# SZU-AdvTech-2024/140-ExtDM-Distribution-Extrapolation-Diffusion-Model-for-Video-Prediction

Hardware: NVIDIA B200
Metric: predicted frames/sec (DDIM, SMMNIST/BAIR 64²) at 1/2/4/8 B200; roofline % (higher is better)
Workload: dtype bf16

## Files before the change

### 140-extdm-distribution-extrapolation-diffusion-model-for-video-prediction_b200/csrc/conv_gemm.cu

```cuda
#include "common.cuh"
#include "../../include/extdm_b200.h"

#include <mutex>
#include <stdio.h>
#include <stdlib.h>
#include <string.h>

namespace extdm {

constexpr int kTileM = 128;
constexpr int kBlockK = 64;
constexpr int kATileBytes = kTileM * kBlockK * 2;
constexpr int kGemmThreads = 192;

struct GemmDev {
  int nk0, nk1, ntaps;
  int box[4], start[4], count[4], ntile[4];
  signed char tap[64][4];
  int n;
  int n_tiles_n, total_tiles;
  void* out;
  int out_fp32;
  long long out_base, out_stride[4];
  int col_group;
  long long col_group_stride;
  const float* bias;
  const void* res;
  int res_fp32;
  long long res_base, res_stride[4];
  const float* col_scale;
  const float* col_shift;
  int act;
  float* gn_part;
  int kh, kw, stages, a_ext_bytes;
  int n_phase;
  long long phase_out[4];
  int tf32;
  int prefetch;
  int dbg;
};

__device__ __forceinline__ float apply_act(float v, int act) {
  if (act == 1) return fmaxf(v, 0.0f);
  if (act == 2) return silu(v);
  if (act == 3) return 1.0f / (1.0f + __expf(-v));
  return v;
}

struct TileCoord {
  int c1, c2, c3, c4, n0, m_tile, phase;
};
__device__ __forceinline__ TileCoord decode_tile(const GemmDev& p, int tile, int BN) {
  TileCoord t;
  const int nt = tile % p.n_tiles_n;
// ... 217 lines not shown
      }
    }
    tc_fence_before();
    __syncwarp();
    if (lane == 0) mbar_arrive(&acc_empty[as]);

    if (GN) {
      asm volatile("bar.sync 1, 128;" ::: "memory");
      if (m < 16)
        p.gn_part[static_cast<long long>(tc.m_tile) * 16 + m] = (sg[m] + sg[16 + m]) + (sg[32 + m] + sg[48 + m]);
    }
  }
}


template <int BN, bool GN, int EPW, int NACC = 2>
__device__ __forceinline__ void epilogue_simple(const GemmDev& p, uint64_t* acc_full, uint64_t* acc_empty, float* s_gn,
                                                uint32_t tmem_base, int warp, int lane) {
  constexpr uint32_t kAccCols = BN < 32 ? 32 : BN;
  constexpr int kChunks = BN / 16;
  constexpr int kGroups = EPW >= NACC ? NACC : (EPW >= 2 ? 2 : 1);
  constexpr int kWpg = EPW / kGroups;
  constexpr int kGThreads = 128 * kWpg;
  const int q = warp & 3;
  const int e = (warp - 2) >> 2;
  const int grp = e / kWpg, eg = e % kWpg;
  float* s_bias = s_gn + grp * 256;
  const int gt = (eg * 4 + ((warp - 2) & 3)) * 32 + lane;
  const int m = q * 32 + lane;
  int r = m;
  const int i1 = r % p.box[0]; r /= p.box[0];
// ... 21 lines not shown
    }
    mbar_wait(&acc_full[as], aphase);
    tc_fence_after();
    const uint32_t taddr = tmem_base + as * kAccCols + (static_cast<uint32_t>(q * 32) << 16);
#pragma unroll 1
    for (int ch = eg; ch < kChunks; ch += kWpg) {
      uint32_t raw[16];
      if (p.dbg & 8) {
#pragma unroll
        for (int j = 0; j < 16; ++j) raw[j] = 0u;
      } else {
        tmem_ld16(taddr + ch * 16, raw);
        tmem_ld_wait();
      }
      float gst[4] = {0.f, 0.f, 0.f, 0.f};
      if (row_ok && n0 + ch * 16 < p.n) {
        float v[16];
#pragma unroll
        for (int j = 0; j < 16; j += 4) {
          const float4 bb = *reinterpret_cast<const float4*>(s_bias + ch * 16 + j);
          v[j] = __uint_as_float(raw[j]) + bb.x; v[j + 1] = __uint_as_float(raw[j + 1]) + bb.y;
          v[j + 2] = __uint_as_float(raw[j + 2]) + bb.z; v[j + 3] = __uint_as_float(raw[j + 3]) + bb.w;
        }
        if (p.act) {
#pragma unroll
          for (int j = 0; j < 16; ++j) v[j] = apply_act(v[j], p.act);
        }
        uint32_t pk[8];
#pragma unroll
        for (int j = 0; j < 8; ++j) pk[j] = pack_bf16(v[2 * j], v[2 * j + 1]);
        if (!(p.dbg & 1)) {
          *reinterpret_cast<uint4*>(orow + ch * 16) = make_uint4(pk[0], pk[1], pk[2], pk[3]);
          *reinterpret_cast<uint4*>(orow + ch * 16 + 8) = make_uint4(pk[4], pk[5], pk[6], pk[7]);
        }
        if (GN) {
#pragma unroll
          for (int j = 0; j < 8; ++j) {
            const float2 f = unpack_bf16(pk[j]);
            gst[j >> 2] += f.x + f.y;
            gst[2 + (j >> 2)] += f.x * f.x + f.y * f.y;
          }
        }
      }
      if (GN && !(p.dbg & 16)) {
        {
          const bool up = (lane & 16) != 0;
          const float s0 = up ? gst[0] : gst[2], k0 = up ? gst[2] : gst[0];
          const float s1 = up ? gst[1] : gst[3], k1 = up ? gst[3] : gst[1];
          gst[0] = k0 + __shfl_xor_sync(0xffffffffu, s0, 16);
          gst[1] = k1 + __shfl_xor_sync(0xffffffffu, s1, 16);
        }
        {
          const bool up = (lane & 8) != 0;
          const float s0 = up ? gst[0] : gst[1], k0 = up ? gst[1] : gst[0];
          gst[0] = k0 + __shfl_xor_sync(0xffffffffu, s0, 8);
        }
        gst[0] += __shfl_xor_sync(0xffffffffu, gst[0], 4);
        gst[0] += __shfl_xor_sync(0xffffffffu, gst[0], 2);
        gst[0] += __shfl_xor_sync(0xffffffffu, gst[0], 1);
        const int cpg = p.n >> 3;
        const int krec = cpg >= 32 ? (cpg >> 4) : 1;
        const int gcol = n0 + ch * 16;
        float* rec = p.gn_part + ((static_cast<long long>(tc.m_tile) * 4 + q) * krec + ((gcol >> 4) & (krec - 1))) * 16;
        const int stat = lane >> 4;
        if (cpg == 8) {
          if ((lane & 7) == 0) rec[stat * 8 + (gcol >> 3) + ((lane >> 3) & 1)] = gst[0];
        } else {
          const float tot = gst[0] + __shfl_xor_sync(0xffffffffu, gst[0], 8);
          if ((lane & 15) == 0) rec[stat * 8 + gcol / cpg] = tot;
        }
      }
    }
    tc_fence_before();
    __syncwarp();
    if (lane == 0) mbar_arrive(&acc_empty[as]);
  }
}

template <int BN, bool SIMPLE>
struct PlainCfg {
  static constexpr int kEpw = SIMPLE ? (BN == 256 ? 4 : 2) : 1;
  static constexpr int kThreads = 64 + 128 * kEpw;
};

template <int BN, int STAGES, bool GN, bool SIMPLE, bool TF32 = false>
__global__ void __launch_bounds__(PlainCfg<BN, SIMPLE>::kThreads, BN == 256 ? 1 : 2)
conv_gemm_kernel(const __grid_constant__ CUtensorMap map_a0, const __grid_constant__ CUtensorMap map_a1,
                 const __grid_constant__ CUtensorMap map_b, const __grid_constant__ GemmDev p) {
  constexpr int kBTileBytes = BN * kBlockK * 2;
  constexpr int kStageBytes = kATileBytes + kBTileBytes;
  constexpr uint32_t kAccCols = BN < 32 ? 32 : BN;
  constexpr uint32_t kTmemCols = 2 * kAccCols;

  extern __shared__ uint8_t smem_raw[];
  uint8_t* smem = reinterpret_cast<uint8_t*>((reinterpret_cast<uintptr_t>(smem_raw) + 1023) & ~uintptr_t(1023));
  uint64_t* full_bar = reinterpret_cast<uint64_t*>(smem + STAGES * kStageBytes);
  uint64_t* empty_bar = full_bar + STAGES;
  uint64_t* acc_full = empty_bar + STAGES;
  uint64_t* acc_empty = acc_full + 2;
  uint32_t* tmem_slot = reinterpret_cast<uint32_t*>(acc_empty + 2);
// ... 95 lines not shown
              for (int k = 0; k < kBlockK / 16; ++k) {
                if (TF32) umma_tf32(tmem_d, da + 2 * k, db + 2 * k, idesc, (it > 0 || k > 0) ? 1u : 0u);
                else umma_bf16(tmem_d, da + 2 * k, db + 2 * k, idesc, (it > 0 || k > 0) ? 1u : 0u);
              }
            }
            umma_commit(&empty_bar[stage]);
          }
          if (++stage == STAGES) { stage = 0; phase ^= 1; }
        }
        if (elect_one()) umma_commit(&acc_full[as]);
      }
    }
    __syncwarp();
  } else {
    if constexpr (SIMPLE)
      epilogue_simple<BN, GN, PlainCfg<BN, SIMPLE>::kEpw>(p, acc_full, acc_empty, s_gn, tmem_base, warp, lane);
    else
      epilogue_loop<BN, GN, false>(p, acc_full, acc_empty, s_gn, tmem_base, warp, lane);
  }

  tc_fence_before();
  __syncthreads();
  if (warp == 1) {
    tc_fence_after();
    tmem_dealloc(tmem_base, kTmemCols);
  }
}


constexpr int kHaloEpw = 4;
constexpr int kHaloThreads = 64 + 128 * kHaloEpw;

template <int BN, bool GN, bool RESB, bool SIMPLE>
__global__ void __launch_bounds__(SIMPLE ? kHaloThreads : kGemmThreads, 1)
conv_halo_kernel(const __grid_constant__ CUtensorMap map_a0, const __grid_constant__ CUtensorMap map_a1,
                 const __grid_constant__ CUtensorMap map_b, const __grid_constant__ GemmDev p) {
  constexpr int kBTileBytes = BN * kBlockK * 2;
  constexpr uint32_t kAccCols = BN < 32 ? 32 : BN;
  constexpr int kAcc = SIMPLE ? (BN <= 64 ? 4 : (BN <= 128 ? 4 : 2)) : 2;
  constexpr uint32_t kTmemCols = kAcc * kAccCols;
  static_assert(kTmemCols <= 512, "TMEM budget");
  constexpr int kMaxStages = 8;

  extern __shared__ uint8_t smem_raw[];
  uint8_t* smem = reinterpret_cast<uint8_t*>((reinterpret_cast<uintptr_t>(smem_raw) + 1023) & ~uintptr_t(1023));
  const int nk = p.nk0 + p.nk1;
  const int ntaps = p.kh * p.kw;
  const int resb_bytes = RESB ? ntaps * nk * kBTileBytes : 0;
// ... 122 lines not shown
                  acc = 1;
                }
              }
              if (p.dbg & 32) mbar_arrive(&empty_bar[stage]); else umma_commit(&empty_bar[stage]);
            }
            accumulate = 1;
            if (++stage == p.stages) { stage = 0; phase ^= 1; }
          }
        }
        if (elect_one()) { if (p.dbg & 32) mbar_arrive(&acc_full[as]); else umma_commit(&acc_full[as]); }
      }
    }
    __syncwarp();
  } else {
    if constexpr (SIMPLE)
      epilogue_simple<BN, GN, kHaloEpw, kAcc>(p, acc_full, acc_empty, s_gn, tmem_base, warp, lane);
    else
      epilogue_loop<BN, GN, false>(p, acc_full, acc_empty, s_gn, tmem_base, warp, lane);
  }

  tc_fence_before();
  __syncthreads();
  if (warp == 1) {
    tc_fence_after();
    tmem_dealloc(tmem_base, kTmemCols);
  }
}

typedef CUresult (*EncodeTiledFn)(CUtensorMap*, CUtensorMapDataType, cuuint32_t, void*, const cuuint64_t*,
                                  const cuuint64_t*, const cuuint32_t*, const cuuint32_t*, CUtensorMapInterleave,
                                  CUtensorMapSwizzle, CUtensorMapL2promotion, CUtensorMapFloatOOBfill);
// ... 35 lines not shown
static int encode_a(CUtensorMap* map, const void* base, int channels, const long long* dim, const long long* stride,
                    const int* box) {
  cuuint64_t dims[5] = {(cuuint64_t)channels, (cuuint64_t)dim[0], (cuuint64_t)dim[1], (cuuint64_t)dim[2],
                        (cuuint64_t)dim[3]};
  cuuint64_t strides[4] = {(cuuint64_t)stride[0] * 2, (cuuint64_t)stride[1] * 2, (cuuint64_t)stride[2] * 2,
                           (cuuint64_t)stride[3] * 2};
  cuuint32_t bx[5] = {(cuuint32_t)kBlockK, (cuuint32_t)box[0], (cuuint32_t)box[1], (cuuint32_t)box[2],
                      (cuuint32_t)box[3]};
  return encode_map(map, base, 5, dims, strides, bx, CU_TENSOR_MAP_L2_PROMOTION_L2_128B);
}

static int sm_count() { return device_sm_count(); }

constexpr int kSmemBudget = 232448 - 4608;

template <int BN, bool GN, bool RESB, bool SIMPLE>
static int launch_halo(const CUtensorMap& ma0, const CUtensorMap& ma1, const CUtensorMap& mb, GemmDev& dev, int m_tiles,
                       int smem_bytes, cudaStream_t stream) {
  static SmemConfigured configured;
  if (!configured.covers(smem_bytes)) {
    cudaError_t e = cudaFuncSetAttribute(conv_halo_kernel<BN, GN, RESB, SIMPLE>, cudaFuncAttributeMaxDynamicSharedMemorySize,
                                         smem_bytes);
    if (e != cudaSuccess) {
      extdm_set_error(cudaGetErrorString(e), __FILE__, __LINE__);
      return EXTDM_ERR_CUDA;
    }
    configured.set(smem_bytes);
  }
  dev.n_tiles_n = (dev.n + BN - 1) / BN;
  dev.total_tiles = m_tiles * dev.n_tiles_n;
  const int resident = sm_count();
  const int grid = dev.total_tiles < resident ? dev.total_tiles : resident;
  conv_halo_kernel<BN, GN, RESB, SIMPLE><<<grid, SIMPLE ? kHaloThreads : kGemmThreads, smem_bytes, stream>>>(ma0, ma1, mb, dev);
  EXTDM_CHECK_LAUNCH();
  return EXTDM_OK;
}

template <int BN, int STAGES, bool GN, bool SIMPLE, bool TF32 = false>
static int launch(const CUtensorMap& ma0, const CUtensorMap& ma1, const CUtensorMap& mb, GemmDev& dev, int m_tiles,
                  cudaStream_t stream) {
  constexpr int kStageBytes = kATileBytes + BN * kBlockK * 2;
  constexpr int smem_bytes = STAGES * kStageBytes + (2 * STAGES + 4) * 8 + 16 + 4096 + 1024;
  static SmemConfigured configured;
  if (!configured.covers(smem_bytes)) {
    cudaError_t e = cudaFuncSetAttribute(conv_gemm_kernel<BN, STAGES, GN, SIMPLE, TF32>,
                                         cudaFuncAttributeMaxDynamicSharedMemorySize, smem_bytes);
    if (e != cudaSuccess) {
      extdm_set_error(cudaGetErrorString(e), __FILE__, __LINE__);
      return EXTDM_ERR_CUDA;
    }
    configured.set(smem_bytes);
  }
  dev.n_tiles_n = (dev.n + BN - 1) / BN;
  dev.total_tiles = m_tiles * dev.n_tiles_n;
  const int resident = sm_count() * (BN == 256 ? 1 : 2);
  const int grid = dev.total_tiles < resident ? dev.total_tiles : resident;
  conv_gemm_kernel<BN, STAGES, GN, SIMPLE, TF32><<<grid, PlainCfg<BN, SIMPLE>::kThreads, smem_bytes, stream>>>(ma0, ma1, mb,
                                                                                                     dev);
  EXTDM_CHECK_LAUNCH();
  return EXTDM_OK;
}

}

extern "C" int extdm_conv_gemm(const ExtdmGemm* g, void* stream_) {
  using namespace extdm;
  cudaStream_t stream = static_cast<cudaStream_t>(stream_);
  if (!g || !g->a0 || !g->w || !g->out) {
    extdm_set_error("extdm_conv_gemm: null operand", __FILE__, __LINE__);
    return EXTDM_ERR_ARG;
  }
  const int n_phase = g->n_phase > 1 ? g->n_phase : 1;
  if (n_phase > 4 || n_phase * g->ntaps > 64 || (n_phase > 1 && (g->gn_partials || g->tf32 || g->w_rows != n_phase * g->n))) {
    extdm_set_error("extdm_conv_gemm: n_phase <= 4, n_phase*ntaps <= 64, w_rows == n_phase*n, no gn_partials / tf32", __FILE__,
                    __LINE__);
    return EXTDM_ERR_ARG;
  }
  if (g->a0_channels <= 0 || g->a0_channels % kBlockK || g->a1_channels % kBlockK || g->ntaps < 1 || g->ntaps > 64 ||
      g->n < 1 || g->box[0] * g->box[1] * g->box[2] * g->box[3] != kTileM || g->col_group < 1) {
    extdm_set_error("extdm_conv_gemm: channels must be multiples of 64, 1..64 taps, box product 128", __FILE__,
                    __LINE__);
    return EXTDM_ERR_ARG;
  }
  GemmDev dev;
  memset(&dev, 0, sizeof dev);
  dev.nk0 = g->a0_channels / kBlockK;
  dev.nk1 = g->a1 ? g->a1_channels / kBlockK : 0;
  dev.ntaps = g->ntaps;
  int m_tiles = 1;
  for (int i = 0; i < 4; ++i) {
    if (g->box[i] < 1 || g->box[i] > 256 || g->count[i] < 1) {
      extdm_set_error("extdm_conv_gemm: bad box/count", __FILE__, __LINE__);
      return EXTDM_ERR_ARG;
    }
    dev.box[i] = g->box[i];
    dev.start[i] = g->start[i];
// ... 9 lines not shown
  dev.out_fp32 = g->out_fp32;
  dev.out_base = g->out_base;
  dev.col_group = g->col_group;
  dev.col_group_stride = g->col_group_stride;
  dev.bias = g->bias;
  dev.res = g->res;
  dev.res_fp32 = g->res_fp32;
  dev.res_base = g->res_base;
  dev.col_scale = g->col_scale;
  dev.col_shift = g->col_shift;
  dev.act = g->act;
  dev.gn_part = g->gn_partials;
  dev.tf32 = g->tf32;
  dev.n_phase = n_phase;
  for (int i = 0; i < 4; ++i) dev.phase_out[i] = (n_phase > 1 && i < n_phase) ? g->phase_out_offset[i] : 0;
  m_tiles *= n_phase;
  static const int dbg_flags = getenv("EXTDM_GEMM_DBG") ? atoi(getenv("EXTDM_GEMM_DBG")) : 0;
  dev.dbg = dbg_flags;
  dev.prefetch = ((dev.nk0 + dev.nk1 >= 2) ? 1 : 0) ^ ((dbg_flags & 64) ? 1 : 0);
  if ((g->col_scale == nullptr) != (g->col_shift == nullptr)) {
    extdm_set_error("extdm_conv_gemm: col_scale and col_shift go together", __FILE__, __LINE__);
    return EXTDM_ERR_ARG;
  }

  int bn = g->block_n;
  if (bn == 0) {
    bn = g->n <= 16 ? 16 : (g->n <= 64 ? 64 : (g->n <= 128 || g->n % 256 ? 128 : 256));
    static const bool no_split = getenv("EXTDM_GEMM_NO_NSPLIT") != nullptr;
    if (!no_split && !g->tf32) {
      const long long ktot_ = static_cast<long long>(g->ntaps) * (dev.nk0 + dev.nk1) * kBlockK;
      const long long slots = (ktot_ >= 4096 ? 1ll : 2ll) * sm_count();
      while (bn > 64 && g->n % (bn / 2) == 0 && static_cast<long long>(m_tiles) * (g->n / (bn / 2)) <= slots) bn /= 2;
    }
  }
  if (n_phase > 1 && g->n % bn) {
    extdm_set_error("extdm_conv_gemm: phases need block_n | n", __FILE__, __LINE__);
    return EXTDM_ERR_ARG;
  }
  if (bn != 16 && bn != 64 && bn != 128 && bn != 256) {
    extdm_set_error("extdm_conv_gemm: block_n must be 16, 64, 128 or 256", __FILE__, __LINE__);
// ... 9 lines not shown
  static const bool halo_off = getenv("EXTDM_NO_HALO") != nullptr;
  static const bool halo7_off = getenv("EXTDM_NO_HALO7") != nullptr;
  static const bool halo_all = getenv("EXTDM_HALO_ALL") != nullptr;
  bool halo = kk && n_phase == 1 && (simple || kk == 7) && !halo_off && !(kk == 7 && halo7_off) &&
              (halo_all || kk == 3 || dev.nk0 + dev.nk1 >= 2) && g->box[2] == 1 && g->box[3] == 1 && g->box[0] % 8 == 0 &&
              (bn == 64 || bn == 128) && !g->tf32;
  int ebox[4] = {g->box[0], g->box[1] + kk - 1, 1, 1};
  bool resb = false;
  int halo_smem = 0;
  if (halo) {
    const int nk = dev.nk0 + dev.nk1;
    const int a_ext = ebox[1] * ebox[0] * 128;
    const int btile = bn * kBlockK * 2;
    const long long resb_bytes = static_cast<long long>(g->ntaps) * nk * btile;
    int stages;
    if (g->n <= bn && resb_bytes + 3ll * a_ext <= kSmemBudget) {
      resb = true;
      stages = static_cast<int>((kSmemBudget - resb_bytes) / a_ext);
    } else {
      stages = kSmemBudget / (a_ext + kk * btile);
    }
    const long long per_kx = a_ext + (resb ? 0 : kk * btile);
    if (stages > 8) stages = 8;
    if (stages < 2) {
      halo = false;
    } else {
      dev.kh = dev.kw = kk;
      dev.stages = stages;
      dev.a_ext_bytes = a_ext;
      halo_smem = static_cast<int>((resb ? resb_bytes : 0) + static_cast<long long>(stages) * per_kx) +
                  (2 * 8 + 10) * 8 + 16 + 4096 + 1024;
// ... 4 lines not shown
  int rc = encode_a(&ma0, g->a0, g->a0_channels, g->a0_dim, g->a0_stride, halo ? ebox : g->box);
  if (rc) return rc;
  if (dev.nk1 > 0) {
    rc = encode_a(&ma1, g->a1, g->a1_channels, g->a1_dim, g->a1_stride, halo ? ebox : g->box);
    if (rc) return rc;
  } else {
    ma1 = ma0;
  }
  const long long ktot = static_cast<long long>(g->ntaps) * (dev.nk0 + dev.nk1) * kBlockK;
  cuuint64_t wd[2] = {(cuuint64_t)ktot, (cuuint64_t)g->w_rows};
  cuuint64_t ws[1] = {(cuuint64_t)ktot * 2};
  cuuint32_t wb[2] = {(cuuint32_t)kBlockK, (cuuint32_t)bn};
  rc = encode_map(&mb, g->w, 2, wd, ws, wb, CU_TENSOR_MAP_L2_PROMOTION_L2_256B);
  if (rc) return rc;

  if (g->gn_partials && ((g->n != 64 && g->n != 128 && g->n != 256 && g->n != 512) || g->n % bn || bn < 64 || !simple ||
                         g->box[3] != 1)) {
    extdm_set_error("extdm_conv_gemm: gn_partials needs n in {64,128,256,512}, block_n | n, a bias-only bf16 epilogue, box[3] == 1",
                    __FILE__, __LINE__);
    return EXTDM_ERR_ARG;
  }
  if (halo) {
    const bool gn = g->gn_partials != nullptr;
#define HALO(BN_, GN_, RB_)                                                                             \
  return simple ? launch_halo<BN_, GN_, RB_, true>(ma0, ma1, mb, dev, m_tiles, halo_smem, stream)      \
                : launch_halo<BN_, GN_, RB_, false>(ma0, ma1, mb, dev, m_tiles, halo_smem, stream)
    if (bn == 64) {
      if (gn) { if (resb) HALO(64, true, true); else HALO(64, true, false); }
      else { if (resb) HALO(64, false, true); else HALO(64, false, false); }
    } else {
      if (gn) { if (resb) HALO(128, true, true); else HALO(128, true, false); }
      else { if (resb) HALO(128, false, true); else HALO(128, false, false); }
    }
#undef HALO
  }
  if (g->gn_partials) {
#define PLAIN(BN_, ST_, GN_)                                                                  \
  return simple ? launch<BN_, ST_, GN_, true>(ma0, ma1, mb, dev, m_tiles, stream)            \
                : launch<BN_, ST_, GN_, false>(ma0, ma1, mb, dev, m_tiles, stream)
    switch (bn) {
      case 64: PLAIN(64, 4, true);
      case 128: PLAIN(128, 3, true);
      default: PLAIN(256, 4, true);
    }
  }
  if (g->tf32) {
    if (g->gn_partials || !g->out_fp32 || g->res || g->col_scale) {
      extdm_set_error("extdm_conv_gemm: tf32 mode supports a bias / activation fp32 epilogue only", __FILE__, __LINE__);
      return EXTDM_ERR_ARG;
    }
// ... 24 lines not shown
```

### 140-extdm-distribution-extrapolation-diffusion-model-for-video-prediction_b200/lib.py

```python
import ctypes as C
import os

_HERE = os.path.dirname(os.path.abspath(__file__))
LIB_PATH = os.environ.get("EXTDM_LIB") or os.path.join(_HERE, "libextdm_b200.so")


class ExtdmGemm(C.Structure):
    _fields_ = [
        ("a0", C.c_void_p), ("a1", C.c_void_p),
        ("a0_channels", C.c_int), ("a1_channels", C.c_int),
        ("a0_dim", C.c_longlong * 4), ("a0_stride", C.c_longlong * 4),
        ("a1_dim", C.c_longlong * 4), ("a1_stride", C.c_longlong * 4),
        ("box", C.c_int * 4), ("start", C.c_int * 4), ("count", C.c_int * 4),
        ("ntaps", C.c_int), ("tap", (C.c_byte * 4) * 64),
        ("w", C.c_void_p), ("n", C.c_int), ("w_rows", C.c_int),
        ("out", C.c_void_p), ("out_fp32", C.c_int), ("out_base", C.c_longlong),
        ("out_stride", C.c_longlong * 4), ("col_group", C.c_int), ("col_group_stride", C.c_longlong),
        ("bias", C.c_void_p),
        ("res", C.c_void_p), ("res_fp32", C.c_int), ("res_base", C.c_longlong), ("res_stride", C.c_longlong * 4),
        ("col_scale", C.c_void_p), ("col_shift", C.c_void_p),
        ("act", C.c_int), ("block_n", C.c_int),
        ("gn_partials", C.c_void_p),
        ("tf32", C.c_int),
        ("n_phase", C.c_int), ("phase_out_offset", C.c_longlong * 4),
    ]


_I, _L, _F, _P = C.c_int, C.c_longlong, C.c_float, C.c_void_p

PROTOTYPES = {
    "extdm_abi_version": [],
    "extdm_last_error": [],
    "extdm_sizeof_gemm": [],
    "extdm_conv_gemm": [C.POINTER(ExtdmGemm), _P],
    "extdm_image_to_cl": [_P, _I, _I, _P, _I, _I, _P, _I, _I, _P, _I, _I, _I, _I, _P],
    "extdm_avgpool2_f32_cl": [_P, _P, _L, _I, _I, _I, _P],
    "extdm_upsample2_f32_cl": [_P, _P, _L, _I, _I, _I, _P],
    "extdm_region_moments": [_P, _I, _I, _I, _I, _I, _I, _F, _P, _P, _P],
    "extdm_pca_affine": [_P, _P, _I, _P],
# ... 98 lines not shown
```

### 140-extdm-distribution-extrapolation-diffusion-model-for-video-prediction_b200/ops.py

```python
import ctypes as C

import torch

from . import lib as _lib

BF16 = torch.bfloat16


class Recorder:

    def __init__(self, record=False):
        self.record = record
        self.steps = []
        self.keep = []
        self.meta = []

    def emit(self, name, args, keep=(), meta=None):
        if self.record:
            self.keep.extend(keep)
            self.steps.append((getattr(_lib.load(), name), args, name))
            self.meta.append(meta or {})
        else:
            _lib.call(name, *args, C.c_void_p(torch.cuda.current_stream().cuda_stream))

# ... 101 lines not shown

def conv3d_taps(k):
    return [(kx - k // 2, ky - k // 2, kt - k // 2) for kt in range(k) for ky in range(k) for kx in range(k)]


def std_box(H, W):
    bw = min(W, 128)
    bh = min(H, 128 // bw)
    bt = 128 // (bw * bh)
    return bw, bh, bt


def gemm(rec, *, a0, c0, dims, strides0, box, start, count, taps, w, n, out, out_stride, out_base=0,
         a1=None, c1=0, strides1=None, out_fp32=False, col_group=None, col_group_stride=0, bias=None,
         res=None, res_fp32=False, res_base=0, res_stride=None, col_scale=None, col_shift=None, act=0,
         block_n=0, gn_partials=None, a1_offset=0, tf32=False, phases=None):
    if phases is not None:
        taps = phases[0][0]
        if any(len(tp) != len(taps) for tp, _ in phases):
            raise ValueError("gemm: every phase needs the same number of taps")
    g = _lib.ExtdmGemm()
    g.a0 = a0.data_ptr()
    g.a1 = 0 if a1 is None else a1.data_ptr() + 2 * a1_offset
    g.a0_channels, g.a1_channels = c0, (c1 if a1 is not None else 0)
    for i in range(4):
        g.a0_dim[i], g.a0_stride[i] = dims[i], strides0[i]
        g.a1_dim[i] = dims[i]
        g.a1_stride[i] = (strides1 or strides0)[i]
        g.box[i], g.start[i], g.count[i] = box[i], start[i], count[i]
        g.out_stride[i] = out_stride[i]
        g.res_stride[i] = (res_stride or out_stride)[i]
    g.ntaps = len(taps)
    all_taps = taps if phases is None else [t for tp, _ in phases for t in tp]
    for i, t in enumerate(all_taps):
        g.tap[i][0], g.tap[i][1], g.tap[i][2], g.tap[i][3] = t[0], t[1], t[2], 0
    n_phase = 1 if phases is None else len(phases)
    g.n_phase = n_phase
    for i in range(n_phase if phases is not None else 0):
        g.phase_out_offset[i] = phases[i][1]
    _chk(w, BF16, "gemm weight")
    if w.shape[1] != len(taps) * (c0 + (c1 if a1 is not None else 0)):
        raise ValueError(f"gemm: weight K {w.shape[1]} != taps*channels {len(taps)}*{c0}+{c1}")
    g.w, g.n, g.w_rows = w.data_ptr(), n, w.shape[0]
    g.out, g.out_fp32, g.out_base = out.data_ptr(), int(out_fp32), out_base
    g.col_group = col_group if col_group else max(n, 1)
    g.col_group_stride = col_group_stride
    g.bias = 0 if bias is None else bias.data_ptr()
    g.res = 0 if res is None else res.data_ptr()
    g.res_fp32, g.res_base = int(res_fp32), res_base
    g.col_scale = 0 if col_scale is None else col_scale.data_ptr()
    g.col_shift = 0 if col_shift is None else col_shift.data_ptr()
    g.act, g.block_n = act, block_n
    g.gn_partials = 0 if gn_partials is None else gn_partials.data_ptr()
    g.tf32 = int(tf32)
# ... 12 lines not shown

def linear_rows(rec, x, w, n, out, *, bias=None, res=None, res_fp32=False, act=0, out_fp32=False, x2=None,
                block_n=0):
    rows, c0 = x.numel() // x.shape[-1], x.shape[-1]
    c1 = 0 if x2 is None else x2.shape[-1]
    ld_out = out.shape[-1]
    gemm(rec, a0=x, c0=c0, a1=x2, c1=c1, dims=(rows, 1, 1, 1), strides0=(c0, rows * c0, rows * c0, rows * c0),
         strides1=None if x2 is None else (c1, rows * c1, rows * c1, rows * c1),
         box=(128, 1, 1, 1), start=(0, 0, 0, 0), count=(rows, 1, 1, 1), taps=[(0, 0, 0)], w=w, n=n, out=out,
         out_stride=(ld_out, 0, 0, 0), out_fp32=out_fp32, bias=bias, res=res, res_fp32=res_fp32,
         res_stride=None if res is None else (res.shape[-1], 0, 0, 0), act=act, block_n=block_n)


def conv_cl(rec, x, w, n, k, out, *, x2=None, bias=None, res=None, res_fp32=False, act=0, out_fp32=False,
            t_range=None, col_scale=None, col_shift=None, out_t_offset=0, res_t_offset=0, taps=None,
            out_scale=1, out_phase=(0, 0), block_n=0, gn_partials=None, x2_t_offset=0, tf32=False, out_pixel_offset=(0, 0)):
    B, T, H, W, c0 = x.shape
    c1 = 0 if x2 is None else x2.shape[-1]
    bw, bh, bt = std_box(H, W)
    t0, t1 = t_range if t_range else (0, T)
    oB, oT, oH, oW, oC = out.shape
    s = out_scale
    ostr = (s * oC, s * oW * oC, oH * oW * oC, oT * oH * oW * oC)
    obase = out_t_offset * oH * oW * oC + ((out_phase[0] + out_pixel_offset[0]) * oW + out_phase[1] + out_pixel_offset[1]) * oC
    rstr, rbase = None, 0
    if res is not None:
        rB, rT, rH, rW, rC = res.shape
        rstr = (rC, rW * rC, rH * rW * rC, rT * rH * rW * rC)
        rbase = res_t_offset * rH * rW * rC
    gemm(rec, a0=x, c0=c0, a1=x2, c1=c1, dims=(W, H, T, B), a1_offset=-x2_t_offset * H * W * c1,
         strides0=(c0, W * c0, H * W * c0, T * H * W * c0),
         strides1=None if x2 is None else (c1, W * c1, H * W * c1, x2.shape[1] * H * W * c1),
         box=(bw, bh, bt, 1), start=(0, 0, t0, 0), count=(W, H, t1 - t0, B),
         taps=taps if taps is not None else conv_taps(k), w=w, n=n, out=out, out_stride=ostr, out_base=obase,
         out_fp32=out_fp32, bias=bias, res=res, res_fp32=res_fp32, res_base=rbase, res_stride=rstr,
         col_scale=col_scale, col_shift=col_shift, act=act, block_n=block_n, gn_partials=gn_partials, tf32=tf32)


def upsample_cl(rec, x, merged, n, out, *, bias=None):
    wm, taps, order = merged
    B, T, H, W, c0 = x.shape
    bw, bh, bt = std_box(H, W)
    oB, oT, oH, oW, oC = out.shape
    gemm(rec, a0=x, c0=c0, dims=(W, H, T, B), strides0=(c0, W * c0, H * W * c0, T * H * W * c0),
         box=(bw, bh, bt, 1), start=(0, 0, 0, 0), count=(W, H, T, B), taps=taps[0], w=wm, n=n, out=out,
         out_stride=(2 * oC, 2 * oW * oC, oH * oW * oC, oT * oH * oW * oC), bias=bias,
         phases=[(taps[i], (py * oW + px) * oC) for i, (py, px) in enumerate(order)])


def pack_conv_weight_f32(w, cin_pad=None, splits=None):
    co, ci, kh, kw = w.shape
# ... 543 lines not shown
```

### 140-extdm-distribution-extrapolation-diffusion-model-for-video-prediction_b200/unet.py

```python
import math

import torch
from torch import nn

from . import composite, ops
from .manifest import UNET_ARCHITECTURES, UnetConfig, is_int_key, unet_manifest
from .paramtree import ParamTree
from .weights import synth_state_dict

BF16 = torch.bfloat16


def _rope_tables(n, dh, device):
    freqs = 1.0 / (10000.0 ** (torch.arange(0, dh, 2, dtype=torch.float32)[: dh // 2] / dh))
    ang = torch.arange(n, dtype=torch.float32)[:, None] * freqs[None, :]
    return ang.cos().contiguous().to(device), ang.sin().contiguous().to(device)


def _t5_rel_bias(emb, T, num_buckets=32, max_distance=32):
    rel = torch.arange(-(T - 1), T)
    n = -rel
    nb = num_buckets // 2
    ret = (n < 0).long() * nb
    n = n.abs()
    max_exact = nb // 2
    large = max_exact + (torch.log(n.float().clamp(min=1) / max_exact) / math.log(max_distance / max_exact)
                         * (nb - max_exact)).long()
    large = torch.minimum(large, torch.full_like(large, nb - 1))
    bucket = ret + torch.where(n < max_exact, n, large)
    return emb.detach().float().cpu()[bucket].t().contiguous()


class PackedUnet:

    def __init__(self, sd, cfg, device):
        self.cfg = cfg
        self.dev = device
        self.f32, self.w = {}, {}
        for k in sd:
            if is_int_key(k) or k.endswith("rotary_emb.freqs"):
                continue
            t = sd[k].detach().to(device=device, dtype=torch.float32)
            if k in ("init_conv.weight", "init_noise_conv.weight") or k.startswith(("time_mlp.", "time_rel_pos_bias.")) \
                    or ".mlp.1." in k or k.endswith("relative_position_bias_table"):
                self.f32[k] = t.contiguous()
# ... 15 lines not shown
            n = w3.shape[0]
            out = torch.zeros(n, 192, device=device, dtype=BF16)
            out[:, :147] = w3[:, :, 0].permute(0, 2, 3, 1).reshape(n, 147).to(BF16)
            return out
        ic = self.f32["init_conv.weight"]
        if cfg.variant in ("base", "u22"):
            self.w["init_flow"] = pack7(ic[:, :3])
            self.w["init_fea"] = ops.pack_conv_weight(ic[:, 3:])
        elif cfg.variant == "u12":
            self.w["init_noise"] = pack7(self.f32["init_noise_conv.weight"])
            self.w["init_full"] = ops.pack_conv_weight(ic)
            self.w["init_fea"] = ops.pack_conv_weight(ic[:, 256:])
            self._pack_composite_init(ic[:, :256, 0])
            c2 = composite.compose_upsampled(ic[:, 256:, 0])
            co = ic.shape[0]
            self.w["init_poly"] = [c2["poly"][i].reshape(co, 25 * 256).to(BF16).contiguous() for i in range(4)]
            for side in ("top", "bottom", "left", "right"):
                self.w["init_fea_" + side] = c2[side].reshape(3 * co, 7 * 256).to(BF16).contiguous()
        else:
            self.w["init_noise"] = pack7(self.f32["init_noise_conv.weight"])
            self.w["init_x"] = ops.pack_conv_weight(ic[:, :256])
            self.w["init_fea"] = ops.pack_conv_weight(ic[:, 256:])
            self._pack_composite_init(ic[:, :256, 0])
        rows, biases, self.ss_off = [], [], {}
        off = 0
        for k in sorted(sd):
            if k.endswith(".mlp.1.weight"):
                p = k[: -len(".mlp.1.weight")]
                self.ss_off[p] = off
                rows.append(self.f32[k])
                biases.append(self.f32[p + ".mlp.1.bias"])
                off += rows[-1].shape[0]
        self.wss = torch.cat(rows, 0).contiguous()
        self.bss = torch.cat(biases, 0).contiguous()
        self.n_ss = off
        self.rel_bias = _t5_rel_bias(sd["time_rel_pos_bias.relative_attention_bias.weight"], cfg.T).to(device)
        self.rope_t = _rope_tables(32, cfg.dim_head, device)
        wd, wh, ww = cfg.window
# ... 372 lines not shown
            x = self._resblock(st, x, "mid_block2", mid)
        else:
            x = self._resblock(st, x, "mid_block2", mid)
            x = self._stw(st, x, "mid_attn2", False)
            x = self._adaptor(st, x, "mid_adaptor")
        self.taps["mid"] = x
        dims = [d] + levels
        in_out = list(zip(dims[:-1], dims[1:]))
        for i, (ci, co) in enumerate(reversed(in_out)):
            p = f"ups.{i}"
            x = self._stage(st, x, p, ci, i > 1, x2=skips.pop())
            if i < nres - 1:
                x = self._upsample(st, x, f"{p}.{rs}")
                self.taps[f"{p}.{rs}"] = x
        if cfg.groups == 8 and d in (64, 128, 256):
            h2f, rf, pf, npart = self._resblock(st, x, "final_conv.0", d, x2=x0, time=False, defer_norm2=True)
            h2o, ro, po, _ = self._resblock(st, x, "occlusion_map.0", d, x2=x0, time=False, defer_norm2=True)
            ops.head_project_gn(st, h2f, rf, pf, pk.f32["final_conv.0.block2.norm.weight"],
                                pk.f32["final_conv.0.block2.norm.bias"], h2o, ro, po,
                                pk.f32["occlusion_map.0.block2.norm.weight"],
                                pk.f32["occlusion_map.0.block2.norm.bias"], npart, pk.f32["final_conv.1.weight"],
                                pk.f32["final_conv.1.bias"], pk.f32["occlusion_map.1.weight"],
                                pk.f32["occlusion_map.1.bias"], self.out, tm)
            return
        hf = self._resblock(st, x, "final_conv.0", d, x2=x0, time=False)
        ho = self._resblock(st, x, "occlusion_map.0", d, x2=x0, time=False)
        ops.head_project(st, hf, ho, pk.f32["final_conv.1.weight"], pk.f32["final_conv.1.bias"],
                         pk.f32["occlusion_map.1.weight"], pk.f32["occlusion_map.1.bias"], self.out, tm)

    def _polyphase_fea(self, rec, fpad, x0):
        cfg, pk, B, H, W = self.cfg, self.pk, self.B, self.H, self.W
        T, tc, tp = cfg.T, cfg.tc, cfg.tp
        d, hw = cfg.dim, H * W
        hp, h = fpad.shape[2], fpad.shape[2] - 4
        top, bottom = self.buf(B, tp, W + 6, 256), self.buf(B, tp, W + 6, 256)
        left, right = self.buf(B, tp, H, 256), self.buf(B, tp, H, 256)
        ops.upsample2_border(rec, fpad, top, bottom, left, right)
        base = tc * hw * d
        for py in range(2):
            for px in range(2):
                ops.gemm(rec, a0=fpad, c0=256, dims=(hp, hp, tp, B), strides0=(256, hp * 256, hp * hp * 256, tp * hp * hp * 256),
                         box=(16, 8, 1, 1), start=(2, 2, 0, 0), count=(h, h, tp, B), taps=ops.conv_taps(5),
                         w=pk.w["init_poly"][py * 2 + px], n=d, out=x0, out_stride=(2 * d, 2 * W * d, hw * d, T * hw * d),
                         out_base=base - 4 * d - 4 * W * d + (py * W + px) * d, bias=pk.f32["init_conv.bias"])
        ostr = (d, W * d, hw * d, T * hw * d)
        for side, a, y0 in (("top", top, 0), ("bottom", bottom, H - 3)):
            taps = [(kx + 3, 0, 0) for kx in range(-3, 4)]
            ops.gemm(rec, a0=a, c0=256, dims=(W + 6, 1, tp, B), strides0=(256, (W + 6) * 256, (W + 6) * 256, tp * (W + 6) * 256),
                     box=(32, 1, 4, 1), start=(0, 0, 0, 0), count=(W, 1, tp, B), taps=taps, w=pk.w["init_fea_" + side], n=d,
                     out=x0, out_stride=ostr, out_base=base + y0 * W * d, res=x0, res_base=base + y0 * W * d, res_stride=ostr,
                     phases=[(taps, pr * W * d) for pr in range(3)])
        for side, a, x_0 in (("left", left, 0), ("right", right, W - 3)):
            taps = [(0, ky, 0) for ky in range(-3, 4)]
            ops.gemm(rec, a0=a, c0=256, dims=(1, H, tp, B), strides0=(256, 256, H * 256, tp * H * 256), box=(1, 32, 4, 1),
                     start=(0, 0, 0, 0), count=(1, H, tp, B), taps=taps, w=pk.w["init_fea_" + side], n=d, out=x0,
                     out_stride=ostr, out_base=base + x_0 * d, res=x0, res_base=base + x_0 * d, res_stride=ostr,
                     phases=[(taps, pr * d) for pr in range(3)])

    def _composite_init(self, rec, x0, res, res_fp32, bias):
# ... 146 lines not shown
```

### include/extdm_b200.h

```cpp
#ifndef EXTDM_B200_H
#define EXTDM_B200_H

#ifdef __cplusplus
extern "C" {
#endif

const char* extdm_last_error(void);
int extdm_abi_version(void);

typedef struct ExtdmGemm {
  const void* a0;
  const void* a1;
  int a0_channels;
  int a1_channels;
  long long a0_dim[4];
  long long a0_stride[4];
  long long a1_dim[4];
  long long a1_stride[4];
  int box[4];
  int start[4];
  int count[4];
  int ntaps;
  signed char tap[64][4];
  const void* w;
// ... 6 lines not shown
  int col_group;
  long long col_group_stride;
  const float* bias;
  const void* res;
  int res_fp32;
  long long res_base;
  long long res_stride[4];
  const float* col_scale;
  const float* col_shift;
  int act;
  int block_n;
  float* gn_partials;
  int tf32;
  int n_phase;
  long long phase_out_offset[4];
} ExtdmGemm;

int extdm_conv_gemm(const ExtdmGemm* g, void* stream);
int extdm_sizeof_gemm(void);


#define EXTDM_GN_CHUNKS 32
int extdm_groupnorm_stats(const void* x, float* stats, int B, long long P, int C, int G, void* stream);

int extdm_groupnorm_apply(const void* x, const float* stats, int n_part, const float* gamma, const float* beta,
                          const float* scale_shift, long long ss_stride, int ss_off, const void* res, void* y,
                          int B, long long P, int C, int G, float eps, void* stream);

int extdm_chan_layernorm(const void* x0, long long x0_outer_stride, int C0, const void* x1,
                         long long x1_outer_stride, int C1, const float* gamma, void* y, long long n_outer,
// ... 158 lines not shown
```

Before: 4252.

## Batch the two output heads' convs and polyphase GEMMs via column-group scatter

Adds a column-group mode to the conv GEMM epilogue, where each group of N columns writes to its own output offset and GroupNorm partial buffer. The two head resblocks (final_conv and occlusion_map) now share one concatenated block1 conv and one res conv instead of running them separately. The polyphase init conv also merges its px pair into a single N=2d GEMM. This cuts kernel launches and reuses the same A-tile loads across both outputs, at the cost of new template instantiations and a fixed BN=128 tile for grouped launches.

```diff
diff --git a/140-extdm-distribution-extrapolation-diffusion-model-for-video-prediction_b200/csrc/conv_gemm.cu b/140-extdm-distribution-extrapolation-diffusion-model-for-video-prediction_b200/csrc/conv_gemm.cu
--- a/140-extdm-distribution-extrapolation-diffusion-model-for-video-prediction_b200/csrc/conv_gemm.cu
+++ b/140-extdm-distribution-extrapolation-diffusion-model-for-video-prediction_b200/csrc/conv_gemm.cu
@@ -38,6 +38,8 @@
   int tf32;
   int prefetch;
   int dbg;
+  int group_n;
+  long long group_out[4], group_gn[4];
 };
 
 __device__ __forceinline__ float apply_act(float v, int act) {
@@ -285,7 +287,7 @@
 }
 
 
-template <int BN, bool GN, int EPW, int NACC = 2>
+template <int BN, bool GN, int EPW, int NACC = 2, bool CG = false>
 __device__ __forceinline__ void epilogue_simple(const GemmDev& p, uint64_t* acc_full, uint64_t* acc_empty, float* s_gn,
                                                 uint32_t tmem_base, int warp, int lane) {
   constexpr uint32_t kAccCols = BN < 32 ? 32 : BN;
@@ -337,6 +339,8 @@
         tmem_ld_wait();
       }
       float gst[4] = {0.f, 0.f, 0.f, 0.f};
+      const int cgrp = CG ? (n0 + ch * 16) / p.group_n : 0;
+      const int gbase = CG ? cgrp * p.group_n : 0;
       if (row_ok && n0 + ch * 16 < p.n) {
         float v[16];
 #pragma unroll
@@ -353,8 +357,10 @@
 #pragma unroll
         for (int j = 0; j < 8; ++j) pk[j] = pack_bf16(v[2 * j], v[2 * j + 1]);
         if (!(p.dbg & 1)) {
-          *reinterpret_cast<uint4*>(orow + ch * 16) = make_uint4(pk[0], pk[1], pk[2], pk[3]);
-          *reinterpret_cast<uint4*>(orow + ch * 16 + 8) = make_uint4(pk[4], pk[5], pk[6], pk[7]);
+          __nv_bfloat16* op = orow + ch * 16;
+          if (CG) op += p.group_out[cgrp] - gbase;
+          *reinterpret_cast<uint4*>(op) = make_uint4(pk[0], pk[1], pk[2], pk[3]);
+          *reinterpret_cast<uint4*>(op + 8) = make_uint4(pk[4], pk[5], pk[6], pk[7]);
         }
         if (GN) {
 #pragma unroll
@@ -381,10 +387,11 @@
         gst[0] += __shfl_xor_sync(0xffffffffu, gst[0], 4);
         gst[0] += __shfl_xor_sync(0xffffffffu, gst[0], 2);
         gst[0] += __shfl_xor_sync(0xffffffffu, gst[0], 1);
-        const int cpg = p.n >> 3;
+        const int cpg = (CG ? p.group_n : p.n) >> 3;
         const int krec = cpg >= 32 ? (cpg >> 4) : 1;
-        const int gcol = n0 + ch * 16;
-        float* rec = p.gn_part + ((static_cast<long long>(tc.m_tile) * 4 + q) * krec + ((gcol >> 4) & (krec - 1))) * 16;
+        const int gcol = n0 + ch * 16 - gbase;
+        float* rec = p.gn_part + (CG ? p.group_gn[cgrp] : 0) +
+                     ((static_cast<long long>(tc.m_tile) * 4 + q) * krec + ((gcol >> 4) & (krec - 1))) * 16;
         const int stat = lane >> 4;
         if (cpg == 8) {
           if ((lane & 7) == 0) rec[stat * 8 + (gcol >> 3) + ((lane >> 3) & 1)] = gst[0];
@@ -406,7 +413,7 @@
   static constexpr int kThreads = 64 + 128 * kEpw;
 };
 
-template <int BN, int STAGES, bool GN, bool SIMPLE, bool TF32 = false>
+template <int BN, int STAGES, bool GN, bool SIMPLE, bool TF32 = false, bool CG = false>
 __global__ void __launch_bounds__(PlainCfg<BN, SIMPLE>::kThreads, BN == 256 ? 1 : 2)
 conv_gemm_kernel(const __grid_constant__ CUtensorMap map_a0, const __grid_constant__ CUtensorMap map_a1,
                  const __grid_constant__ CUtensorMap map_b, const __grid_constant__ GemmDev p) {
@@ -532,7 +539,7 @@
     __syncwarp();
   } else {
     if constexpr (SIMPLE)
-      epilogue_simple<BN, GN, PlainCfg<BN, SIMPLE>::kEpw>(p, acc_full, acc_empty, s_gn, tmem_base, warp, lane);
+      epilogue_simple<BN, GN, PlainCfg<BN, SIMPLE>::kEpw, 2, CG>(p, acc_full, acc_empty, s_gn, tmem_base, warp, lane);
     else
       epilogue_loop<BN, GN, false>(p, acc_full, acc_empty, s_gn, tmem_base, warp, lane);
   }
@@ -549,7 +556,7 @@
 constexpr int kHaloEpw = 4;
 constexpr int kHaloThreads = 64 + 128 * kHaloEpw;
 
-template <int BN, bool GN, bool RESB, bool SIMPLE>
+template <int BN, bool GN, bool RESB, bool SIMPLE, bool CG = false>
 __global__ void __launch_bounds__(SIMPLE ? kHaloThreads : kGemmThreads, 1)
 conv_halo_kernel(const __grid_constant__ CUtensorMap map_a0, const __grid_constant__ CUtensorMap map_a1,
                  const __grid_constant__ CUtensorMap map_b, const __grid_constant__ GemmDev p) {
@@ -702,7 +709,7 @@
     __syncwarp();
   } else {
     if constexpr (SIMPLE)
-      epilogue_simple<BN, GN, kHaloEpw, kAcc>(p, acc_full, acc_empty, s_gn, tmem_base, warp, lane);
+      epilogue_simple<BN, GN, kHaloEpw, kAcc, CG>(p, acc_full, acc_empty, s_gn, tmem_base, warp, lane);
     else
       epilogue_loop<BN, GN, false>(p, acc_full, acc_empty, s_gn, tmem_base, warp, lane);
   }
@@ -768,12 +775,12 @@
 
 constexpr int kSmemBudget = 232448 - 4608;
 
-template <int BN, bool GN, bool RESB, bool SIMPLE>
+template <int BN, bool GN, bool RESB, bool SIMPLE, bool CG = false>
 static int launch_halo(const CUtensorMap& ma0, const CUtensorMap& ma1, const CUtensorMap& mb, GemmDev& dev, int m_tiles,
                        int smem_bytes, cudaStream_t stream) {
   static SmemConfigured configured;
   if (!configured.covers(smem_bytes)) {
-    cudaError_t e = cudaFuncSetAttribute(conv_halo_kernel<BN, GN, RESB, SIMPLE>, cudaFuncAttributeMaxDynamicSharedMemorySize,
+    cudaError_t e = cudaFuncSetAttribute(conv_halo_kernel<BN, GN, RESB, SIMPLE, CG>, cudaFuncAttributeMaxDynamicSharedMemorySize,
                                          smem_bytes);
     if (e != cudaSuccess) {
       extdm_set_error(cudaGetErrorString(e), __FILE__, __LINE__);
@@ -785,19 +792,19 @@
   dev.total_tiles = m_tiles * dev.n_tiles_n;
   const int resident = sm_count();
   const int grid = dev.total_tiles < resident ? dev.total_tiles : resident;
-  conv_halo_kernel<BN, GN, RESB, SIMPLE><<<grid, SIMPLE ? kHaloThreads : kGemmThreads, smem_bytes, stream>>>(ma0, ma1, mb, dev);
+  conv_halo_kernel<BN, GN, RESB, SIMPLE, CG><<<grid, SIMPLE ? kHaloThreads : kGemmThreads, smem_bytes, stream>>>(ma0, ma1, mb, dev);
   EXTDM_CHECK_LAUNCH();
   return EXTDM_OK;
 }
 
-template <int BN, int STAGES, bool GN, bool SIMPLE, bool TF32 = false>
+template <int BN, int STAGES, bool GN, bool SIMPLE, bool TF32 = false, bool CG = false>
 static int launch(const CUtensorMap& ma0, const CUtensorMap& ma1, const CUtensorMap& mb, GemmDev& dev, int m_tiles,
                   cudaStream_t stream) {
   constexpr int kStageBytes = kATileBytes + BN * kBlockK * 2;
   constexpr int smem_bytes = STAGES * kStageBytes + (2 * STAGES + 4) * 8 + 16 + 4096 + 1024;
   static SmemConfigured configured;
   if (!configured.covers(smem_bytes)) {
-    cudaError_t e = cudaFuncSetAttribute(conv_gemm_kernel<BN, STAGES, GN, SIMPLE, TF32>,
+    cudaError_t e = cudaFuncSetAttribute(conv_gemm_kernel<BN, STAGES, GN, SIMPLE, TF32, CG>,
                                          cudaFuncAttributeMaxDynamicSharedMemorySize, smem_bytes);
     if (e != cudaSuccess) {
       extdm_set_error(cudaGetErrorString(e), __FILE__, __LINE__);
@@ -809,7 +816,7 @@
   dev.total_tiles = m_tiles * dev.n_tiles_n;
   const int resident = sm_count() * (BN == 256 ? 1 : 2);
   const int grid = dev.total_tiles < resident ? dev.total_tiles : resident;
-  conv_gemm_kernel<BN, STAGES, GN, SIMPLE, TF32><<<grid, PlainCfg<BN, SIMPLE>::kThreads, smem_bytes, stream>>>(ma0, ma1, mb,
+  conv_gemm_kernel<BN, STAGES, GN, SIMPLE, TF32, CG><<<grid, PlainCfg<BN, SIMPLE>::kThreads, smem_bytes, stream>>>(ma0, ma1, mb,
                                                                                                      dev);
   EXTDM_CHECK_LAUNCH();
   return EXTDM_OK;
@@ -834,6 +841,14 @@
       g->n < 1 || g->box[0] * g->box[1] * g->box[2] * g->box[3] != kTileM || g->col_group < 1) {
     extdm_set_error("extdm_conv_gemm: channels must be multiples of 64, 1..64 taps, box product 128", __FILE__,
                     __LINE__);
+    return EXTDM_ERR_ARG;
+  }
+  const int n_groups = g->n_groups > 1 ? g->n_groups : 1;
+  if (n_groups > 1 &&
+      (n_groups > 4 || g->n % n_groups || (g->n / n_groups) % 16 || n_phase > 1 || g->tf32 || g->res || g->col_scale ||
+       g->out_fp32 || g->col_group < g->n || (g->block_n && g->block_n != 128))) {
+    extdm_set_error("extdm_conv_gemm: column groups need n_groups <= 4 equal groups of a multiple of 16 columns, a bias(+act)"
+                    " bf16 epilogue without col_group, block_n 128, no n_phase / tf32", __FILE__, __LINE__);
     return EXTDM_ERR_ARG;
   }
   GemmDev dev;
@@ -873,6 +888,11 @@
   dev.tf32 = g->tf32;
   dev.n_phase = n_phase;
   for (int i = 0; i < 4; ++i) dev.phase_out[i] = (n_phase > 1 && i < n_phase) ? g->phase_out_offset[i] : 0;
+  dev.group_n = g->n / n_groups;
+  for (int i = 0; i < n_groups && n_groups > 1; ++i) {
+    dev.group_out[i] = g->group_out_offset[i];
+    dev.group_gn[i] = g->group_gn_offset[i];
+  }
   m_tiles *= n_phase;
   static const int dbg_flags = getenv("EXTDM_GEMM_DBG") ? atoi(getenv("EXTDM_GEMM_DBG")) : 0;
   dev.dbg = dbg_flags;
@@ -883,6 +903,7 @@
   }
 
   int bn = g->block_n;
+  if (bn == 0 && n_groups > 1) bn = 128;
   if (bn == 0) {
     bn = g->n <= 16 ? 16 : (g->n <= 64 ? 64 : (g->n <= 128 || g->n % 256 ? 128 : 256));
     static const bool no_split = getenv("EXTDM_GEMM_NO_NSPLIT") != nullptr;
@@ -922,7 +943,7 @@
     const int btile = bn * kBlockK * 2;
     const long long resb_bytes = static_cast<long long>(g->ntaps) * nk * btile;
     int stages;
-    if (g->n <= bn && resb_bytes + 3ll * a_ext <= kSmemBudget) {
+    if (g->n <= bn && n_groups == 1 && resb_bytes + 3ll * a_ext <= kSmemBudget) {
       resb = true;
       stages = static_cast<int>((kSmemBudget - resb_bytes) / a_ext);
     } else {
@@ -957,14 +978,19 @@
   rc = encode_map(&mb, g->w, 2, wd, ws, wb, CU_TENSOR_MAP_L2_PROMOTION_L2_256B);
   if (rc) return rc;
 
-  if (g->gn_partials && ((g->n != 64 && g->n != 128 && g->n != 256 && g->n != 512) || g->n % bn || bn < 64 || !simple ||
+  const int gn_n = dev.group_n;
+  if (g->gn_partials && ((gn_n != 64 && gn_n != 128 && gn_n != 256 && gn_n != 512) || g->n % bn || bn < 64 || !simple ||
                          g->box[3] != 1)) {
-    extdm_set_error("extdm_conv_gemm: gn_partials needs n in {64,128,256,512}, block_n | n, a bias-only bf16 epilogue, box[3] == 1",
+    extdm_set_error("extdm_conv_gemm: gn_partials needs n (per column group) in {64,128,256,512}, block_n | n, a bias-only bf16 epilogue, box[3] == 1",
                     __FILE__, __LINE__);
     return EXTDM_ERR_ARG;
   }
   if (halo) {
     const bool gn = g->gn_partials != nullptr;
+    if (n_groups > 1) {
+      if (gn) return launch_halo<128, true, false, true, true>(ma0, ma1, mb, dev, m_tiles, halo_smem, stream);
+      return launch_halo<128, false, false, true, true>(ma0, ma1, mb, dev, m_tiles, halo_smem, stream);
+    }
 #define HALO(BN_, GN_, RB_)                                                                             \
   return simple ? launch_halo<BN_, GN_, RB_, true>(ma0, ma1, mb, dev, m_tiles, halo_smem, stream)      \
                 : launch_halo<BN_, GN_, RB_, false>(ma0, ma1, mb, dev, m_tiles, halo_smem, stream)
@@ -977,6 +1003,10 @@
     }
 #undef HALO
   }
+  if (n_groups > 1) {
+    if (g->gn_partials) return launch<128, 3, true, true, false, true>(ma0, ma1, mb, dev, m_tiles, stream);
+    return launch<128, 3, false, true, false, true>(ma0, ma1, mb, dev, m_tiles, stream);
+  }
   if (g->gn_partials) {
 #define PLAIN(BN_, ST_, GN_)                                                                  \
   return simple ? launch<BN_, ST_, GN_, true>(ma0, ma1, mb, dev, m_tiles, stream)            \
diff --git a/140-extdm-distribution-extrapolation-diffusion-model-for-video-prediction_b200/lib.py b/140-extdm-distribution-extrapolation-diffusion-model-for-video-prediction_b200/lib.py
--- a/140-extdm-distribution-extrapolation-diffusion-model-for-video-prediction_b200/lib.py
+++ b/140-extdm-distribution-extrapolation-diffusion-model-for-video-prediction_b200/lib.py
@@ -23,6 +23,7 @@
         ("gn_partials", C.c_void_p),
         ("tf32", C.c_int),
         ("n_phase", C.c_int), ("phase_out_offset", C.c_longlong * 4),
+        ("n_groups", C.c_int), ("group_out_offset", C.c_longlong * 4), ("group_gn_offset", C.c_longlong * 4),
     ]
 
 
diff --git a/140-extdm-distribution-extrapolation-diffusion-model-for-video-prediction_b200/ops.py b/140-extdm-distribution-extrapolation-diffusion-model-for-video-prediction_b200/ops.py
--- a/140-extdm-distribution-extrapolation-diffusion-model-for-video-prediction_b200/ops.py
+++ b/140-extdm-distribution-extrapolation-diffusion-model-for-video-prediction_b200/ops.py
@@ -139,7 +139,7 @@
 def gemm(rec, *, a0, c0, dims, strides0, box, start, count, taps, w, n, out, out_stride, out_base=0,
          a1=None, c1=0, strides1=None, out_fp32=False, col_group=None, col_group_stride=0, bias=None,
          res=None, res_fp32=False, res_base=0, res_stride=None, col_scale=None, col_shift=None, act=0,
-         block_n=0, gn_partials=None, a1_offset=0, tf32=False, phases=None):
+         block_n=0, gn_partials=None, a1_offset=0, tf32=False, phases=None, groups=None):
     if phases is not None:
         taps = phases[0][0]
         if any(len(tp) != len(taps) for tp, _ in phases):
@@ -163,6 +163,9 @@
     g.n_phase = n_phase
     for i in range(n_phase if phases is not None else 0):
         g.phase_out_offset[i] = phases[i][1]
+    g.n_groups = 0 if groups is None else len(groups)
+    for i, (oo, go) in enumerate(groups or ()):
+        g.group_out_offset[i], g.group_gn_offset[i] = oo, go
     _chk(w, BF16, "gemm weight")
     if w.shape[1] != len(taps) * (c0 + (c1 if a1 is not None else 0)):
         raise ValueError(f"gemm: weight K {w.shape[1]} != taps*channels {len(taps)}*{c0}+{c1}")
@@ -205,7 +208,8 @@
 
 def conv_cl(rec, x, w, n, k, out, *, x2=None, bias=None, res=None, res_fp32=False, act=0, out_fp32=False,
             t_range=None, col_scale=None, col_shift=None, out_t_offset=0, res_t_offset=0, taps=None,
-            out_scale=1, out_phase=(0, 0), block_n=0, gn_partials=None, x2_t_offset=0, tf32=False, out_pixel_offset=(0, 0)):
+            out_scale=1, out_phase=(0, 0), block_n=0, gn_partials=None, x2_t_offset=0, tf32=False, out_pixel_offset=(0, 0),
+            groups=None):
     B, T, H, W, c0 = x.shape
     c1 = 0 if x2 is None else x2.shape[-1]
     bw, bh, bt = std_box(H, W)
@@ -225,7 +229,8 @@
          box=(bw, bh, bt, 1), start=(0, 0, t0, 0), count=(W, H, t1 - t0, B),
          taps=taps if taps is not None else conv_taps(k), w=w, n=n, out=out, out_stride=ostr, out_base=obase,
          out_fp32=out_fp32, bias=bias, res=res, res_fp32=res_fp32, res_base=rbase, res_stride=rstr,
-         col_scale=col_scale, col_shift=col_shift, act=act, block_n=block_n, gn_partials=gn_partials, tf32=tf32)
+         col_scale=col_scale, col_shift=col_shift, act=act, block_n=block_n, gn_partials=gn_partials, tf32=tf32,
+         groups=groups)
 
 
 def upsample_cl(rec, x, merged, n, out, *, bias=None):
diff --git a/140-extdm-distribution-extrapolation-diffusion-model-for-video-prediction_b200/unet.py b/140-extdm-distribution-extrapolation-diffusion-model-for-video-prediction_b200/unet.py
--- a/140-extdm-distribution-extrapolation-diffusion-model-for-video-prediction_b200/unet.py
+++ b/140-extdm-distribution-extrapolation-diffusion-model-for-video-prediction_b200/unet.py
@@ -29,6 +29,9 @@
     large = torch.minimum(large, torch.full_like(large, nb - 1))
     bucket = ret + torch.where(n < max_exact, n, large)
     return emb.detach().float().cpu()[bucket].t().contiguous()
+
+
+_HEADS = ("final_conv.0", "occlusion_map.0")
 
 
 class PackedUnet:
@@ -74,7 +77,9 @@
             self._pack_composite_init(ic[:, :256, 0])
             c2 = composite.compose_upsampled(ic[:, 256:, 0])
             co = ic.shape[0]
-            self.w["init_poly"] = [c2["poly"][i].reshape(co, 25 * 256).to(BF16).contiguous() for i in range(4)]
+            poly = [c2["poly"][i].reshape(co, 25 * 256).to(BF16) for i in range(4)]
+            self.w["init_poly"] = [torch.cat(poly[2 * py: 2 * py + 2], 0).contiguous() for py in range(2)]
+            self.f32["init_poly_bias"] = self.f32["init_conv.bias"].repeat(2).contiguous()
             for side in ("top", "bottom", "left", "right"):
                 self.w["init_fea_" + side] = c2[side].reshape(3 * co, 7 * 256).to(BF16).contiguous()
         else:
@@ -82,6 +87,10 @@
             self.w["init_x"] = ops.pack_conv_weight(ic[:, :256])
             self.w["init_fea"] = ops.pack_conv_weight(ic[:, 256:])
             self._pack_composite_init(ic[:, :256, 0])
+        if cfg.groups == 8 and cfg.dim == 64:
+            for name in ("block1.proj.weight", "block1.proj.bias", "res_conv.weight", "res_conv.bias"):
+                src = self.w if name.endswith("weight") else self.f32
+                src["heads." + name] = torch.cat([src[f"{h}.{name}"] for h in _HEADS], 0).contiguous()
         rows, biases, self.ss_off = [], [], {}
         off = 0
         for k in sorted(sd):
@@ -484,8 +493,11 @@
                 x = self._upsample(st, x, f"{p}.{rs}")
                 self.taps[f"{p}.{rs}"] = x
         if cfg.groups == 8 and d in (64, 128, 256):
-            h2f, rf, pf, npart = self._resblock(st, x, "final_conv.0", d, x2=x0, time=False, defer_norm2=True)
-            h2o, ro, po, _ = self._resblock(st, x, "occlusion_map.0", d, x2=x0, time=False, defer_norm2=True)
+            if "heads.block1.proj.weight" in pk.w:
+                (h2f, rf, pf, npart), (h2o, ro, po, _) = self._head_blocks(st, x, x0)
+            else:
+                h2f, rf, pf, npart = self._resblock(st, x, "final_conv.0", d, x2=x0, time=False, defer_norm2=True)
+                h2o, ro, po, _ = self._resblock(st, x, "occlusion_map.0", d, x2=x0, time=False, defer_norm2=True)
             ops.head_project_gn(st, h2f, rf, pf, pk.f32["final_conv.0.block2.norm.weight"],
                                 pk.f32["final_conv.0.block2.norm.bias"], h2o, ro, po,
                                 pk.f32["occlusion_map.0.block2.norm.weight"],
@@ -498,6 +510,31 @@
         ops.head_project(st, hf, ho, pk.f32["final_conv.1.weight"], pk.f32["final_conv.1.bias"],
                          pk.f32["occlusion_map.1.weight"], pk.f32["occlusion_map.1.bias"], self.out, tm)
 
+    def _head_blocks(self, rec, x, x0):
+        cfg, pk = self.cfg, self.pk
+        B, T, H, W, _ = x.shape
+        d = cfg.dim
+        plane = B * T * H * W * d
+        npart = ops.gn_parts_per_sample(T, H, W, d)
+        nws = self.gn_ws.numel()
+        ws = torch.zeros(2 * nws, device=self.dev, dtype=torch.float32)
+        h1 = self.buf(2, B, T, H, W, d)
+        ops.conv_cl(rec, x, pk.w["heads.block1.proj.weight"], 2 * d, 3, h1[0], x2=x0, bias=pk.f32["heads.block1.proj.bias"],
+                    gn_partials=ws, groups=[(0, 0), (plane, nws)])
+        r = self.buf(2, B, T, H, W, d)
+        ops.conv_cl(rec, x, pk.w["heads.res_conv.weight"], 2 * d, 1, r[0], x2=x0, bias=pk.f32["heads.res_conv.bias"],
+                    groups=[(0, 0), (plane, 0)])
+        out = []
+        for i, p in enumerate(_HEADS):
+            ops.groupnorm_silu(rec, h1[i], ws[i * nws:], pk.f32[p + ".block1.norm.weight"], pk.f32[p + ".block1.norm.bias"],
+                               h1[i], groups=cfg.groups, n_part=npart)
+            h2 = self.buf(B, T, H, W, d)
+            gnp = torch.zeros_like(self.gn_ws)
+            ops.conv_cl(rec, h1[i], pk.w[p + ".block2.proj.weight"], d, 3, h2, bias=pk.f32[p + ".block2.proj.bias"],
+                        gn_partials=gnp)
+            out.append((h2, r[i], gnp, npart))
+        return out
+
     def _polyphase_fea(self, rec, fpad, x0):
         cfg, pk, B, H, W = self.cfg, self.pk, self.B, self.H, self.W
         T, tc, tp = cfg.T, cfg.tc, cfg.tp
@@ -508,11 +545,10 @@
         ops.upsample2_border(rec, fpad, top, bottom, left, right)
         base = tc * hw * d
         for py in range(2):
-            for px in range(2):
-                ops.gemm(rec, a0=fpad, c0=256, dims=(hp, hp, tp, B), strides0=(256, hp * 256, hp * hp * 256, tp * hp * hp * 256),
-                         box=(16, 8, 1, 1), start=(2, 2, 0, 0), count=(h, h, tp, B), taps=ops.conv_taps(5),
-                         w=pk.w["init_poly"][py * 2 + px], n=d, out=x0, out_stride=(2 * d, 2 * W * d, hw * d, T * hw * d),
-                         out_base=base - 4 * d - 4 * W * d + (py * W + px) * d, bias=pk.f32["init_conv.bias"])
+            ops.gemm(rec, a0=fpad, c0=256, dims=(hp, hp, tp, B), strides0=(256, hp * 256, hp * hp * 256, tp * hp * hp * 256),
+                     box=(16, 8, 1, 1), start=(2, 2, 0, 0), count=(h, h, tp, B), taps=ops.conv_taps(5),
+                     w=pk.w["init_poly"][py], n=2 * d, out=x0, out_stride=(2 * d, 2 * W * d, hw * d, T * hw * d),
+                     out_base=base - 4 * d - 4 * W * d + py * W * d, bias=pk.f32["init_poly_bias"])
         ostr = (d, W * d, hw * d, T * hw * d)
         for side, a, y0 in (("top", top, 0), ("bottom", bottom, H - 3)):
             taps = [(kx + 3, 0, 0) for kx in range(-3, 4)]
diff --git a/include/extdm_b200.h b/include/extdm_b200.h
--- a/include/extdm_b200.h
+++ b/include/extdm_b200.h
@@ -44,6 +44,9 @@
   int tf32;
   int n_phase;
   long long phase_out_offset[4];
+  int n_groups;
+  long long group_out_offset[4];
+  long long group_gn_offset[4];
 } ExtdmGemm;
 
 int extdm_conv_gemm(const ExtdmGemm* g, void* stream);
```

After: 4342, median of 6. +2.1%, better.
